# beast-dev/beast-mcmc

Hardware: NVIDIA H100
Metric: tree log-likelihood evals/sec (higher is better)
Workload: dtype f64

## Files before the change

beast-mcmc_b200/csrc/api.cu:

```cuda
#include "../../include/libhmsbeagle_b200.h"
#include "engine.h"
#include "multi.h"

#include <algorithm>
#include <atomic>
#include <chrono>
#include <cmath>
#include <cstdio>
#include <cstdlib>
#include <cstring>
#include <string>
#include <unordered_map>

using namespace b200;

namespace {

std::mutex gMutex;
std::vector<Instance*> gInstances;

const long kSupportedFlags =
    BEAGLE_FLAG_PRECISION_DOUBLE | BEAGLE_FLAG_PRECISION_SINGLE | BEAGLE_FLAG_COMPUTATION_SYNCH | BEAGLE_FLAG_EIGEN_REAL |
    BEAGLE_FLAG_EIGEN_COMPLEX | BEAGLE_FLAG_SCALING_MANUAL | BEAGLE_FLAG_SCALING_DYNAMIC |
    BEAGLE_FLAG_SCALERS_RAW | BEAGLE_FLAG_SCALERS_LOG | BEAGLE_FLAG_VECTOR_NONE | BEAGLE_FLAG_THREADING_NONE |
    BEAGLE_FLAG_PROCESSOR_GPU | BEAGLE_FLAG_FRAMEWORK_CUDA | BEAGLE_FLAG_PARALLELOPS_GRID |
    BEAGLE_FLAG_PREORDER_TRANSPOSE_AUTO;

int envInt(const char* name, int dflt) {
    const char* v = getenv(name);
    return v ? atoi(v) : dflt;
}

int flushPending(Instance* in);

Instance* getInstance(int id) {
    std::lock_guard<std::mutex> lock(gMutex);
    if (id < 0 || id >= (int)gInstances.size()) return nullptr;
    return gInstances[id];
}

#define SH(id, expr)                                                                         \
    do {                                                                                     \
        Instance* p__ = getInstance(id);                                                     \
        if (p__ != nullptr && p__->shard != nullptr) {                                       \
            Sharded* sh = static_cast<Sharded*>(p__->shard);                                 \
            (void)sh;                                                                        \
            return (expr);                                                                   \
        }                                                                                    \
    } while (0)

#define GET_INSTANCE_LAZY(in, id)                                       \
    Instance* in = getInstance(id);                                     \
    if (in == nullptr) return BEAGLE_ERROR_UNINITIALIZED_INSTANCE;      \
    if (in->shard != nullptr) return BEAGLE_ERROR_NO_IMPLEMENTATION;    \
    if (cudaSetDevice(in->device) != cudaSuccess) return BEAGLE_ERROR_GENERAL;

#define GET_INSTANCE(in, id)                                            \
    GET_INSTANCE_LAZY(in, id)                                           \
    if (!in->pendingMats.empty() || !in->pendingOps.empty()) {          \
        const int flushRc__ = flushPending(in);                         \
        if (flushRc__ != BEAGLE_SUCCESS) return flushRc__;              \
    }

#define CUDA_OK(expr)                                                                        \
    do {                                                                                     \
        cudaError_t e__ = (expr);                                                            \
        if (e__ != cudaSuccess) {                                                            \
            if (getenv("B200_BEAGLE_DEBUG"))                                                 \
                fprintf(stderr, "[b200-beagle] %s failed: %s (%s:%d)\n", #expr,              \
                        cudaGetErrorString(e__), __FILE__, __LINE__);                        \
            return e__ == cudaErrorMemoryAllocation ? BEAGLE_ERROR_OUT_OF_MEMORY             \
                                                    : BEAGLE_ERROR_GENERAL;                  \
        }                                                                                    \
    } while (0)

struct TimedScope {
    Instance* in;
    int cls;
    cudaEvent_t a = nullptr, b = nullptr;
    TimedScope(Instance* i, int c, int kernels = 1) : in(i), cls(c) {
        if (in->timing) {
            in->timedLaunches[cls] += kernels - 1;
            cudaEventCreate(&a);
            cudaEventCreate(&b);
            cudaEventRecord(a, in->stream);
        }
    }
    ~TimedScope() {
        if (in->timing) {
            cudaEventRecord(b, in->stream);
            in->timed[cls].push_back({a, b});
        }
    }
};

void* stage(Instance* in, const void* src, size_t bytes) {
    size_t need = (bytes + 255) & ~size_t(255);
    if (need > in->stageSize) return nullptr;
    if (in->stagePos + need > in->stageSize) {
        cudaStreamSynchronize(in->stream);
        in->stagePos = 0;
    }
    char* h = in->hStage + in->stagePos;
    char* d = in->dStage + in->stagePos;
    memcpy(h, src, bytes);
    if (cudaMemcpyAsync(d, h, bytes, cudaMemcpyHostToDevice, in->stream) != cudaSuccess) return nullptr;
    in->stagePos += need;
    return d;
}

int uploadSmall(Instance* in, void* dDst, const void* src, size_t bytes) {
    size_t need = (bytes + 255) & ~size_t(255);
    if (need > in->stageSize) return BEAGLE_ERROR_OUT_OF_RANGE;
    if (in->stagePos + need > in->stageSize) {
        cudaStreamSynchronize(in->stream);
        in->stagePos = 0;
    }
    char* h = in->hStage + in->stagePos;
    memcpy(h, src, bytes);
    in->stagePos += need;
    CUDA_OK(cudaMemcpyAsync(dDst, h, bytes, cudaMemcpyHostToDevice, in->stream));
    return BEAGLE_SUCCESS;
}

char* ensurePartials(Instance* in, int idx) {
    if (in->partials[idx] == nullptr) {
        if (in->nextSlot >= in->nSlots) return nullptr;
        in->slotOf[idx] = in->nextSlot++;
        in->partials[idx] = in->partialsBase + (size_t)in->slotOf[idx] * in->partialsElems * in->elemBytes();
    }
    return in->partials[idx];
}

bool validRange(int idx, int n) { return idx >= 0 && idx < n; }

void destroyInstance(Instance* in) {
    if (in->shard != nullptr) { shardedDestroy(in); delete in; return; }
    cudaSetDevice(in->device);
    exchangeRelease(in);
    if (in->stream) cudaStreamSynchronize(in->stream);
    cudaFree(in->partialsBase); cudaFree(in->states8Base); cudaFree(in->states32Base);
    for (CachedPlan& cp : in->planCache) { cp.dropGraph(); cudaFree(cp.dBlock); }
    cudaFree(in->dEigen); cudaFree(in->dMat); cudaFree(in->dEvec); cudaFree(in->dIncSums); cudaFree(in->dIncCounter);
    cudaFree(in->dRecipe);
    if (in->hMapped) cudaFreeHost(in->hMapped); cudaFree(in->dRates); cudaFree(in->dWeights);
    cudaFree(in->dFreqs); cudaFree(in->dScale); cudaFree(in->dPatternWeights);
    cudaFree(in->dPatternPartitions); cudaFree(in->dSite); cudaFree(in->dBlockSums); cudaFree(in->dOut);
    cudaFree(in->dCounter); cudaFree(in->dStage); cudaFree(in->dScratch);
    if (in->hStage) cudaFreeHost(in->hStage);
    if (in->hOut) cudaFreeHost(in->hOut);
    for (int c = 0; c < T_CLASSES; ++c)
        for (auto& ev : in->timed[c]) { cudaEventDestroy(ev.first); cudaEventDestroy(ev.second); }
    if (in->stream) cudaStreamDestroy(in->stream);
    delete in;
}

std::vector<BeagleResource> gResources;
std::vector<int> gShardDevices;
int gShardResource = -1;
std::vector<std::string> gResourceStrings;
BeagleResourceList gResourceList = {nullptr, 0};
std::once_flag gResourceOnce;

void buildResources() {
    int n = 0;
    if (cudaGetDeviceCount(&n) != cudaSuccess) { cudaGetLastError(); n = 0; }
    gResourceStrings.reserve(2 * (n + 1));
    gResourceStrings.push_back("CPU (host)");
    gResourceStrings.push_back("no host implementation in this library | use a GPU resource (1..N)");
    for (int d = 0; d < n; ++d) {
        cudaDeviceProp prop;
        if (cudaGetDeviceProperties(&prop, d) != cudaSuccess) { cudaGetLastError(); continue; }
        char buf[512];
        snprintf(buf, sizeof buf, "%s", prop.name);
        gResourceStrings.push_back(buf);
        snprintf(buf, sizeof buf, "Global memory (MB): %zu | SMs: %d | compute capability: %d.%d | "
                 "native walk kernels (sm_90a), fp64 arithmetic, fp64 or fp32 (4-state) partials",
                 (size_t)(prop.totalGlobalMem >> 20), prop.multiProcessorCount, prop.major, prop.minor);
        gResourceStrings.push_back(buf);
    }
    gShardDevices.clear();
    if (const char* env = getenv("B200_SHARD_DEVICES")) {
        for (const char* q = env; *q;) {
            char* end = nullptr;
            const long d = strtol(q, &end, 10);
            if (end == q) break;
            if (d >= 0 && d < n) gShardDevices.push_back((int)d);
            q = (*end == ',') ? end + 1 : end;
        }
    } else {
        for (int d = 0; d < n; ++d) gShardDevices.push_back(d);
    }
    if (gShardDevices.size() > (size_t)kMaxGroup) gShardDevices.resize(kMaxGroup);
    if (!gShardDevices.empty()) {
        char buf[512];
        snprintf(buf, sizeof buf, "GPU x %zu (pattern-sharded)", gShardDevices.size());
        gResourceStrings.push_back(buf);
        snprintf(buf, sizeof buf, "one instance over %zu GPUs | contiguous pattern blocks (Patterns.java:142-169 rule) | "
                 "per-shard sums added over NVLink inside the root kernel", gShardDevices.size());
        gResourceStrings.push_back(buf);
        gShardResource = (int)(gResourceStrings.size() / 2) - 1;
    }
    size_t count = gResourceStrings.size() / 2;
// ... 966 lines not shown
    in->planCache.reserve(16);
    in->thinR1 = envInt("B200_THIN_R1", 1);
    in->stackTail = envInt("B200_STACK_TAIL", 0);
    in->phaseT = envInt("B200_PHASE_T", 0);
    in->phaseTmin = std::max(1, envInt("B200_PHASE_TMIN", 4));
    in->phaseSmall = envInt("B200_PHASE_SMALL", 24);
    in->phaseOversub = std::max(0, envInt("B200_PHASE_OVERSUB", 0));
    in->walkMinBlocks = envInt("B200_WALK_MINB", 4);
    in->walkMinBlocksSet = getenv("B200_WALK_MINB") != nullptr;
    in->tensorR = envInt("B200_TENSOR_R", 2) >= 4 ? 4 : 2;
    in->genericMma = envInt("B200_GENERIC_MMA", 1);
    in->mmaWarps = envInt("B200_MMA_WARPS", 4) == 8 ? 8 : 4;
    cudaDeviceProp prop;
    bool ok = cudaGetDeviceProperties(&prop, in->device) == cudaSuccess;
    if (ok) { in->smCount = prop.multiProcessorCount; in->maxSmemOptin = prop.sharedMemPerBlockOptin; }
    in->walkR = envInt("B200_WALK_R", 4);
    if (in->walkR != 1 && in->walkR != 2 && in->walkR != 4 && in->walkR != 8) in->walkR = 4;
    if (getenv("B200_WALK_R") == nullptr && in->matCP > 0) {
        const int G = 32 / in->matCP;
        while (in->walkR > 1 && (in->Ppad + G * in->walkR - 1) / (G * in->walkR) < in->smCount) in->walkR >>= 1;
    }
    in->stackDepthMax = std::min(64, std::max(0, envInt("B200_STACK_DEPTH", 12)));
    if (single) { in->walkVariant = 0; in->stackTail = 0; }

    ok = ok && cudaStreamCreateWithFlags(&in->stream, cudaStreamNonBlocking) == cudaSuccess;
    const size_t eigenStride = 2 * (size_t)in->S * in->S + 2 * in->S;
    const size_t matElems = (size_t)in->nMatrices * in->matStride;
    const int rootBlocks = (in->Ppad + 255) / 256;
    in->stageSize = size_t(8) << 20;
    auto alloc = [&](auto** p, size_t elems) {
        if (!ok) return;
        using T = std::remove_pointer_t<std::remove_pointer_t<decltype(p)>>;
        size_t bytes = std::max<size_t>(elems, 1) * sizeof(T);
        ok = cudaMalloc(reinterpret_cast<void**>(p), bytes) == cudaSuccess &&
             cudaMemsetAsync(*p, 0, bytes, in->stream) == cudaSuccess;
    };
    alloc(&in->dEigen, std::max(1, in->nEigen) * eigenStride);
    alloc(&in->dMat, matElems);
    if (in->matCP > 0) alloc(&in->dEvec, (size_t)in->nMatrices * in->matCP * 4);
    if (in->matCP > 0 && in->matCP <= 8 && in->virtualCherries) {
        alloc(&in->dRecipe, (size_t)in->nBuffers * 32 * in->matCP);
        in->cherryTip1.assign(in->nBuffers, -1);
        in->cherryTip2.assign(in->nBuffers, -1);
        in->cherryStored.assign(in->nBuffers, 0);
    }
    if (in->matCP > 0 && in->matCP <= 8) {
        alloc(&in->dIncSums, (size_t)in->Ppad / 4 + 8);
        alloc(&in->dIncCounter, 4);
        in->fuseSmall = envInt("B200_FUSE", 1);
        if (ok && in->fuseSmall) {
            if (cudaHostAlloc(reinterpret_cast<void**>(&in->hMapped), 64, cudaHostAllocMapped) == cudaSuccess &&
                cudaHostGetDevicePointer(reinterpret_cast<void**>(&in->dMapped), in->hMapped, 0) == cudaSuccess) {
                memset(in->hMapped, 0, 64);
            } else {
                cudaGetLastError();
                if (in->hMapped) cudaFreeHost(in->hMapped);
                in->hMapped = nullptr;
            }
        }
    }
    alloc(&in->dRates, (size_t)in->nSets * in->C);
    alloc(&in->dWeights, (size_t)in->nSets * in->C);
    alloc(&in->dFreqs, (size_t)in->nSets * in->Sp);
    alloc(&in->dScale, (size_t)in->nScale * in->Ppad);
    alloc(&in->dPatternWeights, in->Ppad);
    alloc(&in->dPatternPartitions, in->Ppad);
    alloc(&in->dSite, in->Ppad);
    alloc(&in->dBlockSums, rootBlocks);
    alloc(&in->dOut, 1024);
    alloc(&in->dCounter, 4);
    alloc(&in->dStage, in->stageSize);
    alloc(&in->states8Base, (size_t)std::max(1, in->tipCount) * in->Ppad);
    alloc(&in->states32Base, (size_t)std::max(1, in->tipCount) * in->Ppad);
    if (ok) {
        int want[2] = {in->nPartials, std::max(1, in->nPartials - std::min(in->nCompact, in->tipCount))};
        for (int attempt = 0; attempt < 2 && in->partialsBase == nullptr; ++attempt) {
            size_t bytes = (size_t)want[attempt] * in->partialsElems * in->elemBytes();
            if (cudaMalloc(reinterpret_cast<void**>(&in->partialsBase), bytes) == cudaSuccess) in->nSlots = want[attempt];
            else { cudaGetLastError(); in->partialsBase = nullptr; }
        }
        if (in->partialsBase == nullptr) { destroyInstance(in); return BEAGLE_ERROR_OUT_OF_MEMORY; }
    }
    ok = ok && cudaMallocHost(reinterpret_cast<void**>(&in->hStage), in->stageSize) == cudaSuccess;
    ok = ok && cudaMallocHost(reinterpret_cast<void**>(&in->hOut), 1024 * sizeof(double)) == cudaSuccess;
    if (ok) {
        in->hRates.assign((size_t)in->nSets * in->C, 1.0);
        in->hWeights.assign((size_t)in->nSets * in->C, 0.0);
        in->hFreqs.assign((size_t)in->nSets * 4, 0.0);
        std::vector<double> ones((size_t)std::max(in->nSets * in->C, in->Ppad), 1.0);
        ok = cudaMemcpyAsync(in->dRates, ones.data(), sizeof(double) * in->nSets * in->C, cudaMemcpyHostToDevice,
                             in->stream) == cudaSuccess;
        std::vector<double> w(in->Ppad, 0.0);
        std::fill(w.begin(), w.begin() + in->P, 1.0);
        ok = ok && cudaMemcpyAsync(in->dPatternWeights, w.data(), sizeof(double) * in->Ppad, cudaMemcpyHostToDevice,
                                   in->stream) == cudaSuccess;
        ok = ok && cudaStreamSynchronize(in->stream) == cudaSuccess;
    }
    if (!ok) {
        cudaError_t e = cudaGetLastError();
        destroyInstance(in);
        return e == cudaErrorMemoryAllocation ? BEAGLE_ERROR_OUT_OF_MEMORY : BEAGLE_ERROR_GENERAL;
    }
    in->partitionCount = 1;
    in->partBegin.assign(1, 0);
    in->partEnd.assign(1, in->P);
    {
        std::lock_guard<std::mutex> lock(gMutex);
        int id = -1;
        for (size_t k = 0; k < gInstances.size(); ++k) if (gInstances[k] == nullptr) { id = (int)k; break; }
        if (id < 0) { gInstances.push_back(nullptr); id = (int)gInstances.size() - 1; }
        gInstances[id] = in;
        in->id = id;
    }
    if (returnInfo != nullptr) {
        returnInfo->resourceNumber = resource;
        returnInfo->resourceName = rl->list[resource].name;
        returnInfo->implName = single ? gImplNameSingle : gImplName;
        returnInfo->implDescription = gImplDesc;
        returnInfo->flags = in->flags;
    }
    return in->id;
}

int beagleFinalizeInstance(int instance) {
    Instance* in = nullptr;
    {
        std::lock_guard<std::mutex> lock(gMutex);
        if (instance < 0 || instance >= (int)gInstances.size() || gInstances[instance] == nullptr)
            return BEAGLE_ERROR_UNINITIALIZED_INSTANCE;
        in = gInstances[instance];
        gInstances[instance] = nullptr;
    }
    destroyInstance(in);
    return BEAGLE_SUCCESS;
}

int beagleFinalize(void) {
    std::vector<Instance*> all;
    {
        std::lock_guard<std::mutex> lock(gMutex);
        all.swap(gInstances);
    }
    for (Instance* in : all) if (in) destroyInstance(in);
    return BEAGLE_SUCCESS;
}

int beagleSetCPUThreadCount(int instance, int) {
    SH(instance, BEAGLE_SUCCESS);
    GET_INSTANCE(in, instance);
    (void)in;
    return BEAGLE_SUCCESS;
}

int beagleSetTipStates(int instance, int tipIndex, const int* inStates) {
    SH(instance, shSetTipStates(sh, tipIndex, inStates));
    GET_INSTANCE(in, instance);
    if (!validRange(tipIndex, in->nBuffers) || inStates == nullptr) return BEAGLE_ERROR_OUT_OF_RANGE;
    std::vector<int> s32(in->Ppad, in->S);
    std::vector<uint8_t> s8(in->Ppad, (uint8_t)in->S);
    for (int p = 0; p < in->P; ++p) {
        int s = inStates[p];
        if (s < 0 || s >= in->S) s = in->S;
        s32[p] = s;
        s8[p] = (uint8_t)s;
    }
    if (tipIndex >= in->tipCount) return BEAGLE_ERROR_OUT_OF_RANGE;
// ... 141 lines not shown
    GET_INSTANCE(in, instance);
    if (!validRange(stateFrequenciesIndex, in->nSets)) return BEAGLE_ERROR_OUT_OF_RANGE;
    std::vector<double> f(in->Sp, 0.0);
    memcpy(f.data(), inStateFrequencies, sizeof(double) * in->S);
    if (in->hFreqs.size() == (size_t)in->nSets * 4 && in->S <= 4)
        for (int i = 0; i < 4; ++i) in->hFreqs[(size_t)stateFrequenciesIndex * 4 + i] = i < in->S ? inStateFrequencies[i] : 0.0;
    return uploadSmall(in, in->dFreqs + (size_t)stateFrequenciesIndex * in->Sp, f.data(), sizeof(double) * in->Sp);
}

int beagleSetCategoryWeights(int instance, int categoryWeightsIndex, const double* inCategoryWeights) {
    SH(instance, shBroadcast(sh, [&](int c) { return beagleSetCategoryWeights(c, categoryWeightsIndex, inCategoryWeights); }));
    GET_INSTANCE(in, instance);
    if (!validRange(categoryWeightsIndex, in->nSets)) return BEAGLE_ERROR_OUT_OF_RANGE;
    std::copy(inCategoryWeights, inCategoryWeights + in->C, in->hWeights.begin() + (size_t)categoryWeightsIndex * in->C);
    return uploadSmall(in, in->dWeights + (size_t)categoryWeightsIndex * in->C, inCategoryWeights, sizeof(double) * in->C);
}

int beagleSetCategoryRatesWithIndex(int instance, int categoryRatesIndex, const double* inCategoryRates) {
    SH(instance, shBroadcast(sh, [&](int c) { return beagleSetCategoryRatesWithIndex(c, categoryRatesIndex, inCategoryRates); }));
    GET_INSTANCE(in, instance);
    if (!validRange(categoryRatesIndex, in->nSets)) return BEAGLE_ERROR_OUT_OF_RANGE;
    std::copy(inCategoryRates, inCategoryRates + in->C, in->hRates.begin() + (size_t)categoryRatesIndex * in->C);
    return uploadSmall(in, in->dRates + (size_t)categoryRatesIndex * in->C, inCategoryRates, sizeof(double) * in->C);
}

int beagleSetCategoryRates(int instance, const double* inCategoryRates) {
    return beagleSetCategoryRatesWithIndex(instance, 0, inCategoryRates);
}

int beagleSetPatternWeights(int instance, const double* inPatternWeights) {
    SH(instance, shSetPatternWeights(sh, inPatternWeights));
    GET_INSTANCE(in, instance);
    std::vector<double> w(in->Ppad, 0.0);
    memcpy(w.data(), inPatternWeights, sizeof(double) * in->P);
    CUDA_OK(cudaMemcpyAsync(in->dPatternWeights, w.data(), sizeof(double) * in->Ppad, cudaMemcpyHostToDevice, in->stream));
    CUDA_OK(cudaStreamSynchronize(in->stream));
    return BEAGLE_SUCCESS;
}

int beagleSetPatternPartitions(int instance, int partitionCount, const int* inPatternPartitions) {
    SH(instance, BEAGLE_ERROR_NO_IMPLEMENTATION);
    GET_INSTANCE(in, instance);
    if (partitionCount < 1 || partitionCount > 1000) return BEAGLE_ERROR_OUT_OF_RANGE;
    std::vector<int> begin(partitionCount, 0), end(partitionCount, 0);
    int prev = -1;
    for (int p = 0; p < in->P; ++p) {
        int k = inPatternPartitions[p];
        if (k < 0 || k >= partitionCount) return BEAGLE_ERROR_OUT_OF_RANGE;
        if (k < prev) return BEAGLE_ERROR_NO_IMPLEMENTATION;
        if (k != prev) { for (int q = prev + 1; q <= k; ++q) begin[q] = end[q] = p; prev = k; }
        end[k] = p + 1;
    }
    for (int q = prev + 1; q < partitionCount; ++q) begin[q] = end[q] = in->P;
    in->bufferEpoch++;
    in->partitionCount = partitionCount;
    in->partBegin = begin;
    in->partEnd = end;
    in->hostPartitions.assign(inPatternPartitions, inPatternPartitions + in->P);
    return BEAGLE_SUCCESS;
}

static int updateMatricesImpl(Instance* in, const int* eigenIndices, int eigenIndexScalar, const int* rateSets,
                              const int* probabilityIndices, const double* edgeLengths, int count) {
    if (count <= 0) return BEAGLE_SUCCESS;
    std::vector<double> block((size_t)count + (3 * (size_t)count + 1) / 2);
    int* pack = reinterpret_cast<int*>(block.data() + count);
    for (int k = 0; k < count; ++k) {
        int e = eigenIndices ? eigenIndices[k] : eigenIndexScalar;
        int r = rateSets ? rateSets[k] : 0;
        if (!validRange(probabilityIndices[k], in->nMatrices) || !validRange(e, in->nEigen) ||
            !validRange(r, in->nSets))
            return BEAGLE_ERROR_OUT_OF_RANGE;
        pack[k] = probabilityIndices[k];
        pack[count + k] = e;
        pack[2 * (size_t)count + k] = r;
    }
    if (in->matCP > 0)
        for (int k = 0; k < count; ++k) {
            const int e = eigenIndices ? eigenIndices[k] : eigenIndexScalar;
            in->matEigen[probabilityIndices[k]] = e;
            in->matEigenGen[probabilityIndices[k]] = in->eigenGen[e];
        }
    memcpy(block.data(), edgeLengths, sizeof(double) * count);
    double* dLen = static_cast<double*>(stage(in, block.data(), sizeof(double) * block.size()));
    if (dLen == nullptr) return BEAGLE_ERROR_OUT_OF_MEMORY;
    int* dIdx = reinterpret_cast<int*>(dLen + count);
    TimedScope ts(in, T_MATRICES);
    CUDA_OK(launchTransitionMatrices(in, dIdx, dIdx + count, dIdx + 2 * (size_t)count, dLen, count));
    return BEAGLE_SUCCESS;
}

}
namespace {
int flushPendingImpl(Instance* in) {
    int rc = BEAGLE_SUCCESS;
    if (!in->pendingMats.empty()) {
        const int n = (int)in->pendingMats.size();
        std::vector<int> eig(n), rate(n), prob(n);
        std::vector<double> len(n);
        for (int k = 0; k < n; ++k) {
            eig[k] = in->pendingMats[k].eigen; rate[k] = in->pendingMats[k].rateSet;
            prob[k] = in->pendingMats[k].prob; len[k] = in->pendingMats[k].len;
        }
        in->pendingMats.clear();
        rc = updateMatricesImpl(in, eig.data(), 0, rate.data(), prob.data(), len.data(), n);
    }
    if (!in->pendingOps.empty()) {
        std::vector<HostOp> hops;
        hops.swap(in->pendingOps);
        const int rc2 = planAndLaunch(in, hops, false);
        if (rc == BEAGLE_SUCCESS) rc = rc2;
    }
    return rc;
}

bool fusionPossible(const Instance* in) {
    return in->fuseSmall && in->matCP > 0 && in->matCP <= 8 && !in->timing && !in->exchangeOn && in->walkVariant == 0 &&
           in->eigenWalk && in->hMapped != nullptr;
}

int launchFused(Instance* in, int E, int wIdx, int fIdx, int cum, double* outSum) {
    IncArgs A;
    memset(&A, 0, sizeof A);
    A.partials = in->partialsBase; A.stride = in->partialsElems; A.states = in->states8Base; A.mats = in->dMat;
    A.evecs = in->dEvec; A.scale = in->dScale; A.matStride = in->matStride;
    A.S = in->S; A.C = in->C; A.Ppad = in->Ppad; A.P = in->P; A.logScalers = in->logScalers ? 1 : 0;
    const double* h = in->hEigen.data() + (size_t)E * 36;
    for (int q = 0; q < 16; ++q) { A.V[q] = h[q]; A.Vi[q] = h[16 + q]; }
    for (int q = 0; q < 4; ++q) A.eval[q] = h[32 + q];
    A.nMats = (int)in->pendingMats.size();
    std::unordered_map<int, int> pendingOf;
    for (int q = 0; q < A.nMats; ++q) {
        A.mat[q] = IncMat{in->pendingMats[q].prob, in->pendingMats[q].rateSet, in->pendingMats[q].len};
        for (int c = 0; c < 8; ++c) A.rate[q][c] = c < in->C ? in->hRates[(size_t)in->pendingMats[q].rateSet * in->C + c] : 0.0;
        pendingOf[in->pendingMats[q].prob] = q;
    }
    A.nOps = (int)in->pendingOps.size();
    {
        std::vector<int> outside;
        for (int k = 0; k < A.nOps; ++k)
            for (int c : {in->pendingOps[k].c1, in->pendingOps[k].c2}) {
                bool written = false;
                for (int w = 0; w < k; ++w) written = written || in->pendingOps[w].dest == c;
                if (!written) outside.push_back(c);
            }
        CUDA_OK(storeCherries(in, outside.data(), (int)outside.size()));
    }
    int prevDest = -1;
    for (int k = 0; k < A.nOps; ++k) {
        const HostOp& o = in->pendingOps[k];
        IncOp& d = A.op[k];
        const bool t1 = in->states32[o.c1] != nullptr, t2 = in->states32[o.c2] != nullptr;
        int c1 = o.c1, c2 = o.c2, m1 = o.m1, m2 = o.m2;
        d.flags = 0;
        if (k > 0 && !t1 && c1 == prevDest) d.flags = 1;
        else if (k > 0 && !t2 && c2 == prevDest) { std::swap(c1, c2); std::swap(m1, m2); d.flags = 1; }
        const bool s1 = in->states32[c1] != nullptr, s2 = in->states32[c2] != nullptr;
        d.dest = in->slotOf[o.dest];
        d.c1 = s1 ? -(c1 + 1) : in->slotOf[c1];
        d.c2 = s2 ? -(c2 + 1) : in->slotOf[c2];
        auto mat = [&](int m) { auto it = pendingOf.find(m); return it == pendingOf.end() ? m : -(it->second + 1); };
        d.m1 = mat(m1); d.m2 = mat(m2);
        d.sw = o.sw; d.sr = o.sw >= 0 ? -1 : o.sr;
        prevDest = o.dest;
    }
    for (int c = 0; c < 8; ++c) A.weights[c] = c < in->C ? in->hWeights[(size_t)wIdx * in->C + c] : 0.0;
    for (int i = 0; i < 4; ++i) A.freqs[i] = in->hFreqs[(size_t)fIdx * 4 + i];
    A.cum = cum == BEAGLE_OP_NONE ? nullptr : in->dScale + (size_t)cum * in->Ppad;
    A.patternWeights = in->dPatternWeights; A.site = in->dSite; A.blockSums = in->dIncSums; A.counter = in->dIncCounter;
// ... 988 lines not shown
```

beast-mcmc_b200/csrc/engine.h:

```cpp
#pragma once
#include <cuda_runtime.h>
#include <cstdint>
#include <mutex>
#include <vector>

namespace b200 {

struct alignas(16) DevOp {
    double* dest;
    const double* c1;
    const double* c2;
    const void* s1;
    const void* s2;
    const double* m1;
    const double* m2;
    double* scaleWrite;
    const double* scaleRead;
    double* cumScale;
    int pBegin, pEnd;
    int srcSlot1, srcSlot2;
    int dstSlot;
    int pad_;
};

// ... 57 lines not shown
    double* site; double* blockSums; unsigned int* counter; double* out;
    volatile double* hostOut; volatile unsigned long long* hostFlag; unsigned long long seq;
    IncMat mat[kIncMaxMats];
    IncOp op[kIncMaxOps];
};

constexpr int kMaxGroup = 16;
struct ExchangeSlot { double value; unsigned long long seq; };
struct Exchange {
    int rank = 0, size = 1;
    unsigned long long seq = 0;
    long long timeoutCycles = 0;
    ExchangeSlot* peers[kMaxGroup] = {};
};

constexpr int kStackSlots = 3;

struct Instance {
    int id = -1, device = 0, resource = 0;
    int tipCount = 0, nPartials = 0, nCompact = 0, S = 0, P = 0, nEigen = 0, nMatrices = 0, C = 0, nScale = 0;
    int Sp = 0, Ppad = 0, nBuffers = 0, nSets = 1;
    long flags = 0;
    bool logScalers = false, complexEigen = false;
    cudaStream_t stream = nullptr;
    int smCount = 132;
    size_t maxSmemOptin = 0;

    bool single = false;
    size_t partialsElems = 0;
    size_t elemBytes() const { return single ? sizeof(float) : sizeof(double); }
    char* partialsBase = nullptr;
    int nSlots = 0, nextSlot = 0;
    std::vector<int> slotOf;
    std::vector<char*> partials;
    uint8_t* states8Base = nullptr;
    int* states32Base = nullptr;
    std::vector<uint8_t*> states8;
    std::vector<int*> states32;
    int matCP = 0;
    size_t matStride = 0;

    double* dEigen = nullptr;
    double* dMat = nullptr;
    double* dEvec = nullptr;
    std::vector<int> matEigen;
    std::vector<unsigned> matEigenGen, eigenGen;
    std::vector<char> eigenReal;
    std::vector<char> eigenKind;
    std::vector<double> hEigen;
    int eigenWalk = 1;
    int tipMode = 2;
    int thinTipMode = 3;
    int virtualCherries = 1;
    std::vector<int> cherryTip1, cherryTip2;
    std::vector<char> cherryStored;
    double* dRecipe = nullptr;
    double* dRates = nullptr;
    std::vector<double> hRates, hWeights, hFreqs;
    double* dWeights = nullptr;
    double* dFreqs = nullptr;
    double* dScale = nullptr;
    std::vector<char> scaleIsLog;
    double* dPatternWeights = nullptr;
    int* dPatternPartitions = nullptr;
    double* dSite = nullptr;
    double* dBlockSums = nullptr;
    double* dOut = nullptr;
    unsigned int* dCounter = nullptr;
    int lookaheadPre = 1;
    int prePhases = 1;
    int useGraphs = 1;
    int lookahead = 1;
    int forward = 1;
    int stackSlots = kStackSlots;
    bool debugLog = false;
    double* dScratch = nullptr;
    size_t scratchDoubles = 0;
    int partitionCount = 1;
    std::vector<int> partBegin, partEnd;
    std::vector<int> hostPartitions;

    char* hStage = nullptr;
    char* dStage = nullptr;
    size_t stageSize = 0, stagePos = 0;
    double* hOut = nullptr;

    int fuseSmall = 1;
    struct PendingMat { int prob, eigen, rateSet; double len; };
    std::vector<PendingMat> pendingMats;
    std::vector<HostOp> pendingOps;
    int pendingCum = -1;
    double* hMapped = nullptr;
    double* dMapped = nullptr;
    double* dIncSums = nullptr;
    unsigned int* dIncCounter = nullptr;
    unsigned long long incSeq = 0;
    long fusedLaunches = 0;

    void* shard = nullptr;
    Exchange exchange;
    ExchangeSlot* dSlots = nullptr;
    std::vector<void*> ipcOpened;
    bool exchangeOn = false;

    bool timing = false;
    std::vector<std::pair<cudaEvent_t, cudaEvent_t>> timed[T_CLASSES];
    double timedMs[T_CLASSES] = {0, 0, 0};
    long timedLaunches[T_CLASSES] = {0, 0, 0};

    size_t walkSmemConfigured = 0, genericSmemConfigured = 0, mmaSmemConfigured[8] = {0, 0, 0, 0, 0, 0, 0, 0};
    int walkBlock = 128;
    int walkVariant = 0;
    std::vector<CachedPlan> planCache;
    int planCacheSize = 4;
    long planClock = 0;
    unsigned long bufferEpoch = 0;
    int reorder = 1;
    int thinR1 = 1;
    int stackTail = 0;
    int stackDepthMax = 12;
    int walkMinBlocks = 4;
    bool walkMinBlocksSet = false;
    int mmaWarps = 4;
    int tensorR = 2;
    int genericMma = 1;
    int walkR = 4;
    int phaseTmin = 4, phaseOversub = 0, phaseSmall = 24;
    int phaseT = 0;
};

struct Sharded;
Instance* instanceById(int id);
void exchangeRelease(Instance* in);
int shardedCreate(Instance* parent, int g, const int* devices, int tipCount, int partialsBufferCount, int compactBufferCount,
                  int stateCount, int patternCount, int eigenBufferCount, int matrixBufferCount, int categoryCount,
                  int scaleBufferCount, long preferenceFlags, long requirementFlags, void* details );
void shardedDestroy(Instance* parent);

cudaError_t launchTransitionMatrices(Instance* in, const int* dProbIdx, const int* dEigenIdx,
                                     const int* dRateSet, const double* dLengths, int count);
cudaError_t launchWalk4(Instance* in, const Op4* dOps, const int4* dSubs, int nSubs, int stackDepth, int maxWindow, bool preOrder);
cudaError_t updateWalk4EGraph(cudaGraphExec_t exec, const std::vector<cudaGraphNode_t>& kernelNodes, const double* eigen);
cudaError_t launchWalk4E(Instance* in, const Op4* dOps, const int4* dSubs, int nSubs, int maxWindow, bool aligned,
                         const double* eigen, const int4* dVirtTips, int stackSlots);
bool walk4pServes(const Instance* in, int nSubs, int maxWindow);
bool walkStackBuilt(const Instance* in);
cudaError_t launchCherrySnapshot(Instance* in, const int4* dItems, int count);
cudaError_t launchCherryStore(Instance* in, const int4* dItems, int count);
cudaError_t launchWalkGeneric(Instance* in, const DevOp* dOps, const int4* dSubs, int nSubs, int maxWindow, bool preOrder);
size_t edgeDerivativeWorkspace(const Instance* in, int count);
cudaError_t launchEdgeDerivatives(Instance* in, const EdgeRefT<void>* dEdges, int count, const double* weights, double* outPerPattern,
                                  double* outSum, double* outSumSq, double* partial);
int compressSitePatterns(int device, int taxa, int sites, const int* hStates, int* hPatternOfSite, int* hPatterns,
                         double* hWeights, int* hPatternCount);
int crossProductBlocks(const Instance* in, int count);
cudaError_t launchCrossProducts(Instance* in, const EdgeRefT<void>* dEdges, int count, const double* rates,
                                const double* weights, double* scratch);
cudaError_t launchRoot(Instance* in, const void* root, const double* weights, const double* freqs,
                       const double* cumScale, int pBegin, int pEnd, double* dOutSlot, const Exchange* exchange = nullptr);
cudaError_t launchIncremental(Instance* in, const IncArgs& args);
cudaError_t launchCombineMatrices(Instance* in, const int* dFirst, const int* dSecond, const int* dResult, int count, bool multiply);
cudaError_t launchExchangeSum(Instance* in, const double* dVals, int n, double* dOutJoint, const Exchange* exchange);
cudaError_t launchScaleAccumulate(Instance* in, const int* dIdx, int count, double* cum, double sign,
                                  int pBegin, int pEnd);
cudaError_t launchRescalePartialsForGet(Instance* in, double* tmp, const double* cum);

// ... 45 lines not shown
```

beast-mcmc_b200/csrc/kernels.cu:

```cuda
#include "engine.h"
#include "walk4.cuh"

#include <algorithm>
#include <cfloat>

namespace b200 {

__device__ __forceinline__ void dmma884acc(double& d0, double& d1, double a, double b) {
    asm("mma.sync.aligned.m8n8k4.row.col.f64.f64.f64.f64 {%0,%1}, {%2}, {%3}, {%0,%1};"
        : "+d"(d0), "+d"(d1) : "d"(a), "d"(b));
}

__global__ void k_transition(const double* __restrict__ eigenBase, size_t eigenStride, int S, int Sp, int C,
                             int complexForm, const double* __restrict__ ratesBase,
                             const int* __restrict__ probIdx, const int* __restrict__ eigenIdx,
                             const int* __restrict__ rateSet, const double* __restrict__ lengths,
                             double* __restrict__ matBase, size_t matStride, int matCP, double* __restrict__ evecBase) {
    extern __shared__ double sm[];
    double* ec = sm;
    double* ss = sm + S;
    int* pt = reinterpret_cast<int*>(sm + 2 * S);
    const int b = blockIdx.x, c = blockIdx.y;
    const double* E = eigenBase + (size_t)eigenIdx[b] * eigenStride;
    const double* evec = E;
    const double* ievc = E + (size_t)S * S;
    const double* eval = E + 2 * (size_t)S * S;
    const double d = lengths[b] * ratesBase[(size_t)rateSet[b] * C + c];
    for (int k = threadIdx.x; k < S; k += blockDim.x) {
        double im = complexForm ? eval[S + k] : 0.0;
        if (im == 0.0) {
            ec[k] = exp(d * eval[k]); ss[k] = 0.0; pt[k] = k;
        } else {
            int run = 0;
            for (int q = k - 1; q >= 0 && eval[S + q] != 0.0; --q) ++run;
            const bool first = (run % 2 == 0);
            int k0 = first ? k : k - 1;
            double bb = eval[S + k0];
            double expat = exp(d * eval[k0]);
            ec[k] = expat * cos(d * bb);
            ss[k] = (first ? 1.0 : -1.0) * expat * sin(d * bb);
            pt[k] = first ? k + 1 : k - 1;
        }
    }
    __syncthreads();
    if (evecBase != nullptr && threadIdx.x < 4)
        evecBase[((size_t)probIdx[b] * matCP + c) * 4 + threadIdx.x] = threadIdx.x < S ? ec[threadIdx.x] : 0.0;
    double* out = matBase + (size_t)probIdx[b] * matStride + (matCP ? (size_t)c * 4 : (size_t)c * Sp * Sp);
    const int rowStride = matCP ? matCP * 4 : Sp;
    for (int idx = threadIdx.x; idx < Sp * Sp; idx += blockDim.x) {
        int j = idx / Sp, i = idx % Sp;
        double acc = 0.0;
        if (i < S && j < S) {
            for (int k = 0; k < S; ++k) {
                double iexp = ec[k] * ievc[(size_t)k * S + j] + ss[k] * ievc[(size_t)pt[k] * S + j];
                acc += evec[(size_t)i * S + k] * iexp;
            }
            acc = fabs(acc);
        }
        out[(size_t)j * rowStride + i] = acc;
        if (!matCP) {
            const size_t ld = (size_t)Sp + 4;
            double* padded = matBase + (size_t)probIdx[b] * matStride + (size_t)C * Sp * Sp;
            padded[((size_t)c * Sp + i) * ld + j] = acc;
            padded[(size_t)C * Sp * ld + ((size_t)c * Sp + j) * ld + i] = acc;
        } else {
            double* mm = matBase + (size_t)probIdx[b] * matStride + 16 * matCP;
            mm[(size_t)c * 32 + i * 4 + j] = acc;
            mm[(size_t)c * 32 + 16 + i * 4 + j] = 0.0;
            double* mt = mm + (size_t)C * 32;
            mt[(size_t)c * 20 + j * 4 + i] = (j < S) ? acc : ((j == S && i < S) ? 1.0 : 0.0);
            if (j == 0) mt[(size_t)c * 20 + 16 + i] = (S == 4 && i < S) ? 1.0 : 0.0;
        }
    }
}

__device__ __forceinline__ size_t matEntry(int matCP, int Sp, int c, int i, int j) {
    return matCP ? ((size_t)j * matCP + c) * 4 + i : ((size_t)c * Sp + j) * Sp + i;
}
__global__ void __launch_bounds__(256)
k_combine_matrices(double* __restrict__ matBase, size_t matStride, int S, int Sp, int C, int matCP,
                   const int* __restrict__ first, const int* __restrict__ second, const int* __restrict__ result, int multiply) {
    const int q = blockIdx.x, c = blockIdx.y;
    const double* A = matBase + (size_t)first[q] * matStride;
    const double* B = matBase + (size_t)second[q] * matStride;
    double* R = matBase + (size_t)result[q] * matStride;
    for (int idx = threadIdx.x; idx < Sp * Sp; idx += blockDim.x) {
        const int i = idx / Sp, j = idx % Sp;
        double v = 0.0;
        if (i < S && j < S) {
            if (multiply) for (int k = 0; k < S; ++k) v += A[matEntry(matCP, Sp, c, i, k)] * B[matEntry(matCP, Sp, c, k, j)];
            else v = A[matEntry(matCP, Sp, c, i, j)] + B[matEntry(matCP, Sp, c, i, j)];
        }
        R[matEntry(matCP, Sp, c, i, j)] = v;
        if (!matCP) {
            const size_t ld = (size_t)Sp + 4;
            double* padded = R + (size_t)C * Sp * Sp;
            padded[((size_t)c * Sp + i) * ld + j] = v;
            padded[(size_t)C * Sp * ld + ((size_t)c * Sp + j) * ld + i] = v;
        } else {
            double* mm = R + 16 * matCP;
            mm[(size_t)c * 32 + i * 4 + j] = v;
            mm[(size_t)c * 32 + 16 + i * 4 + j] = 0.0;
            double* mt = mm + (size_t)C * 32;
            mt[(size_t)c * 20 + j * 4 + i] = (j < S) ? v : ((j == S && i < S) ? 1.0 : 0.0);
            if (j == 0) mt[(size_t)c * 20 + 16 + i] = (S == 4 && i < S) ? 1.0 : 0.0;
        }
    }
}

cudaError_t launchCombineMatrices(Instance* in, const int* dFirst, const int* dSecond, const int* dResult, int count, bool multiply) {
    if (count <= 0) return cudaSuccess;
    k_combine_matrices<<<dim3(count, in->C), 256, 0, in->stream>>>(in->dMat, in->matStride, in->S, in->Sp, in->C, in->matCP,
                                                                   dFirst, dSecond, dResult, multiply ? 1 : 0);
    return cudaGetLastError();
}

template <int NT>
__global__ void __launch_bounds__(128)
k_transition_mma(const double* __restrict__ eigenBase, size_t eigenStride, int S, int C,
                 const double* __restrict__ ratesBase, const int* __restrict__ probIdx,
                 const int* __restrict__ eigenIdx, const int* __restrict__ rateSet,
                 const double* __restrict__ lengths, double* __restrict__ matBase, size_t matStride) {
    constexpr int Sp = 8 * NT;
    constexpr int LD = Sp + 4;
    extern __shared__ double smt[];
    double* As = smt;
    double* Bt = smt + Sp * LD;
    double* ex = Bt + Sp * LD;
    const int b = blockIdx.x, c = blockIdx.y, tid = threadIdx.x;
    const double* E = eigenBase + (size_t)eigenIdx[b] * eigenStride;
    const double* evec = E;
    const double* ievc = E + (size_t)S * S;
    const double* eval = E + 2 * (size_t)S * S;
    const double d = lengths[b] * ratesBase[(size_t)rateSet[b] * C + c];
    for (int k = tid; k < Sp; k += 128) ex[k] = k < S ? exp(d * eval[k]) : 0.0;
    __syncthreads();
    for (int q = tid; q < Sp * Sp; q += 128) {
        const int r = q / Sp, col = q % Sp;
        As[r * LD + col] = (r < S && col < S) ? evec[(size_t)r * S + col] : 0.0;
        Bt[col * LD + r] = (r < S && col < S) ? ievc[(size_t)r * S + col] * ex[r] : 0.0;
    }
    __syncthreads();
    const int lane = tid & 31, w = tid >> 5, g = lane >> 2, t = lane & 3;
    double* outT = matBase + (size_t)probIdx[b] * matStride + (size_t)c * Sp * Sp;
    double* outR = matBase + (size_t)probIdx[b] * matStride + (size_t)C * Sp * Sp + (size_t)c * Sp * LD;
    double* outTp = outR + (size_t)C * Sp * LD;
    for (int mt = w; mt < NT; mt += 4) {
        double acc[NT][2];
#pragma unroll
        for (int n = 0; n < NT; ++n) { acc[n][0] = 0.0; acc[n][1] = 0.0; }
        const double* arow = As + (8 * mt + g) * LD + t;
        const double* brow = Bt + g * LD + t;
#pragma unroll 4
        for (int kc = 0; kc < Sp / 4; ++kc) {
            const double a = arow[4 * kc];
#pragma unroll
            for (int n = 0; n < NT; ++n) dmma884acc(acc[n][0], acc[n][1], a, brow[n * 8 * LD + 4 * kc]);
        }
        const int i = 8 * mt + g;
#pragma unroll
        for (int n = 0; n < NT; ++n) {
            const int j = 8 * n + 2 * t;
            const double v0 = fabs(acc[n][0]), v1 = fabs(acc[n][1]);
            *reinterpret_cast<double2*>(outR + (size_t)i * LD + j) = make_double2(v0, v1);
            outT[(size_t)j * Sp + i] = v0;
            outT[(size_t)(j + 1) * Sp + i] = v1;
            outTp[(size_t)j * LD + i] = v0;
            outTp[(size_t)(j + 1) * LD + i] = v1;
        }
    }
}

template <int NT>
static cudaError_t launchTransitionMmaT(Instance* in, const int* dProbIdx, const int* dEigenIdx, const int* dRateSet,
                                        const double* dLengths, int count) {
    constexpr int Sp = 8 * NT;
    const size_t smem = (2 * (size_t)Sp * (Sp + 4) + Sp) * sizeof(double);
    static_assert(Sp <= 64, "shared-memory budget");
    cudaError_t e = cudaFuncSetAttribute(k_transition_mma<NT>, cudaFuncAttributeMaxDynamicSharedMemorySize, (int)smem);
    if (e != cudaSuccess) return e;
    dim3 grid(count, in->C);
    k_transition_mma<NT><<<grid, 128, smem, in->stream>>>(in->dEigen, 2 * (size_t)in->S * in->S + 2 * in->S, in->S, in->C,
                                                          in->dRates, dProbIdx, dEigenIdx, dRateSet, dLengths, in->dMat,
                                                          in->matStride);
    return cudaGetLastError();
}

cudaError_t launchTransitionMatrices(Instance* in, const int* dProbIdx, const int* dEigenIdx,
                                     const int* dRateSet, const double* dLengths, int count) {
    if (count <= 0) return cudaSuccess;
    if (in->genericMma && in->matCP == 0 && !in->complexEigen) {
        switch (in->Sp / 8) {
            case 1: return launchTransitionMmaT<1>(in, dProbIdx, dEigenIdx, dRateSet, dLengths, count);
            case 2: return launchTransitionMmaT<2>(in, dProbIdx, dEigenIdx, dRateSet, dLengths, count);
            case 3: return launchTransitionMmaT<3>(in, dProbIdx, dEigenIdx, dRateSet, dLengths, count);
            case 4: return launchTransitionMmaT<4>(in, dProbIdx, dEigenIdx, dRateSet, dLengths, count);
            case 8: return launchTransitionMmaT<8>(in, dProbIdx, dEigenIdx, dRateSet, dLengths, count);
            default: break;
        }
    }
    size_t smem = (size_t)in->S * (2 * sizeof(double) + sizeof(int)) + 16;
    int threads = in->Sp * in->Sp >= 1024 ? 256 : (in->Sp * in->Sp >= 128 ? 128 : 32);
    dim3 grid(count, in->C);
    k_transition<<<grid, threads, smem, in->stream>>>(in->dEigen, 2 * (size_t)in->S * in->S + 2 * in->S, in->S,
                                                      in->Sp, in->C, in->complexEigen ? 1 : 0, in->dRates,
                                                      dProbIdx, dEigenIdx, dRateSet, dLengths, in->dMat,
                                                      in->matStride, in->matCP, in->matCP ? in->dEvec : nullptr);
    return cudaGetLastError();
}

struct Mat4 { double r[4][4]; };

template <int CP>
__device__ __forceinline__ void loadMat(const double* __restrict__ m, Mat4& M) {
    ldg256_ro(m, M.r[0]); ldg256_ro(m + 4 * CP, M.r[1]); ldg256_ro(m + 8 * CP, M.r[2]); ldg256_ro(m + 12 * CP, M.r[3]);
}

__device__ __forceinline__ void applyMat(const Mat4& M, const double (&x)[4], double (&y)[4]) {
#pragma unroll
    for (int i = 0; i < 4; ++i) y[i] = M.r[0][i] * x[0] + M.r[1][i] * x[1] + M.r[2][i] * x[2] + M.r[3][i] * x[3];
}

template <typename T, int CP, int R, bool STACK, bool FIRST>
__device__ __forceinline__ void childTerm(const WalkArgs& A, int child, int matIdx, int slot, int moff, size_t off0,
                                          int p0, bool catValid, int pBegin, int pEnd, const double2* stackMem,
                                          int nthreads, double (&y)[R][4]) {
    constexpr int G = 32 / CP;
    const int S = A.S;
    const double* m = A.mats + (size_t)matIdx * A.matStride + moff;
    if (child < 0) {
        const uint8_t* t = A.states + (size_t)(-child - 1) * A.Ppad;
#pragma unroll
        for (int r = 0; r < R; ++r) {
            const int p = p0 + r * G;
            const bool active = catValid && p >= pBegin && p < pEnd;
            const int s = active ? (int)__ldg(t + p) : S;
            double v[4];
            if (s < S) ldg256_ro(m + 4 * CP * s, v);
            else {
#pragma unroll
                for (int i = 0; i < 4; ++i) v[i] = (i < S) ? 1.0 : 0.0;
            }
#pragma unroll
            for (int i = 0; i < 4; ++i) y[r][i] = FIRST ? v[i] : y[r][i] * v[i];
        }
    } else {
        Mat4 M;
        loadMat<CP>(m, M);
        const T* xg = static_cast<const T*>(A.partials) + (size_t)child * A.stride + off0;
#pragma unroll
        for (int r = 0; r < R; ++r) {
            const int p = p0 + r * G;
            const bool active = catValid && p >= pBegin && p < pEnd;
            double x[4], v[4];
            if (STACK && slot != 0xFF) {
                double2 lo = stackMem[((slot * R + r) * 2 + 0) * nthreads + threadIdx.x];
                double2 hi = stackMem[((slot * R + r) * 2 + 1) * nthreads + threadIdx.x];
                x[0] = lo.x; x[1] = lo.y; x[2] = hi.x; x[3] = hi.y;
            } else if (active) {
                loadCell(xg + (size_t)r * G * 4, x);
            } else { x[0] = x[1] = x[2] = x[3] = 0.0; }
            applyMat(M, x, v);
#pragma unroll
            for (int i = 0; i < 4; ++i) y[r][i] = FIRST ? v[i] : y[r][i] * v[i];
        }
    }
}

template <typename T, int CP, int R, bool STACK, bool PRE>
__device__ __forceinline__ void walk4Body(const WalkArgs& A) {
    static_assert(sizeof(T) == 8 || !STACK, "the operand-stack variant is built for fp64 partials only");
    constexpr int G = 32 / CP;
    extern __shared__ double2 stackMem[];
    const int lane = threadIdx.x & 31;
    const int warp = (blockIdx.x * blockDim.x + threadIdx.x) >> 5;
    const int c = lane / G;
    const int4 range = __ldg(A.subs + blockIdx.y);
    const int p0 = range.z + warp * (G * R) + (lane % G);
    if (range.z + warp * (G * R) >= range.w) return;
    const bool catValid = c < A.C;
    const int cc = catValid ? c : 0;
    const size_t off0 = ((size_t)cc * A.Ppad + p0) * 4;
    const int moff = cc * 4;
    const int nthreads = blockDim.x;
    const int last = range.y - 1;

    Op4 cur = loadOp(A.ops + range.x);
    double d[R][4];
#pragma unroll
    for (int r = 0; r < R; ++r) d[r][0] = d[r][1] = d[r][2] = d[r][3] = 0.0;
// ... 1717 lines not shown
```

Before: 2578.

## Add quad-per-matrix transition kernel for 4-state compact layout and zero-copy index staging

Result: faster. 2666, median of 6 (+3.4%).

```diff
diff --git a/beast-mcmc_b200/csrc/api.cu b/beast-mcmc_b200/csrc/api.cu
--- a/beast-mcmc_b200/csrc/api.cu
+++ b/beast-mcmc_b200/csrc/api.cu
@@ -94,7 +94,7 @@
     }
 };
 
-void* stage(Instance* in, const void* src, size_t bytes) {
+static char* stageHost(Instance* in, const void* src, size_t bytes) {
     size_t need = (bytes + 255) & ~size_t(255);
     if (need > in->stageSize) return nullptr;
     if (in->stagePos + need > in->stageSize) {
@@ -102,23 +102,27 @@
         in->stagePos = 0;
     }
     char* h = in->hStage + in->stagePos;
-    char* d = in->dStage + in->stagePos;
-    memcpy(h, src, bytes);
-    if (cudaMemcpyAsync(d, h, bytes, cudaMemcpyHostToDevice, in->stream) != cudaSuccess) return nullptr;
-    in->stagePos += need;
-    return d;
-}
-
-int uploadSmall(Instance* in, void* dDst, const void* src, size_t bytes) {
-    size_t need = (bytes + 255) & ~size_t(255);
-    if (need > in->stageSize) return BEAGLE_ERROR_OUT_OF_RANGE;
-    if (in->stagePos + need > in->stageSize) {
-        cudaStreamSynchronize(in->stream);
-        in->stagePos = 0;
-    }
-    char* h = in->hStage + in->stagePos;
     memcpy(h, src, bytes);
     in->stagePos += need;
+    return h;
+}
+
+void* stage(Instance* in, const void* src, size_t bytes) {
+    char* h = stageHost(in, src, bytes);
+    if (h == nullptr) return nullptr;
+    char* d = in->dStage + (h - in->hStage);
+    if (cudaMemcpyAsync(d, h, bytes, cudaMemcpyHostToDevice, in->stream) != cudaSuccess) return nullptr;
+    return d;
+}
+
+static const void* stageMapped(Instance* in, const void* src, size_t bytes) {
+    char* h = stageHost(in, src, bytes);
+    return h == nullptr ? nullptr : in->hStageDev + (h - in->hStage);
+}
+
+int uploadSmall(Instance* in, void* dDst, const void* src, size_t bytes) {
+    char* h = stageHost(in, src, bytes);
+    if (h == nullptr) return BEAGLE_ERROR_OUT_OF_RANGE;
     CUDA_OK(cudaMemcpyAsync(dDst, h, bytes, cudaMemcpyHostToDevice, in->stream));
     return BEAGLE_SUCCESS;
 }
@@ -1251,6 +1255,7 @@
         if (in->partialsBase == nullptr) { destroyInstance(in); return BEAGLE_ERROR_OUT_OF_MEMORY; }
     }
     ok = ok && cudaMallocHost(reinterpret_cast<void**>(&in->hStage), in->stageSize) == cudaSuccess;
+    ok = ok && cudaHostGetDevicePointer(reinterpret_cast<void**>(&in->hStageDev), in->hStage, 0) == cudaSuccess;
     ok = ok && cudaMallocHost(reinterpret_cast<void**>(&in->hOut), 1024 * sizeof(double)) == cudaSuccess;
     if (ok) {
         in->hRates.assign((size_t)in->nSets * in->C, 1.0);
@@ -1558,9 +1563,11 @@
             in->matEigenGen[probabilityIndices[k]] = in->eigenGen[e];
         }
     memcpy(block.data(), edgeLengths, sizeof(double) * count);
-    double* dLen = static_cast<double*>(stage(in, block.data(), sizeof(double) * block.size()));
+    const size_t blockBytes = sizeof(double) * block.size();
+    const double* dLen = static_cast<const double*>(in->matCP > 0 ? stageMapped(in, block.data(), blockBytes)
+                                                                   : stage(in, block.data(), blockBytes));
     if (dLen == nullptr) return BEAGLE_ERROR_OUT_OF_MEMORY;
-    int* dIdx = reinterpret_cast<int*>(dLen + count);
+    const int* dIdx = reinterpret_cast<const int*>(dLen + count);
     TimedScope ts(in, T_MATRICES);
     CUDA_OK(launchTransitionMatrices(in, dIdx, dIdx + count, dIdx + 2 * (size_t)count, dLen, count));
     return BEAGLE_SUCCESS;
diff --git a/beast-mcmc_b200/csrc/engine.h b/beast-mcmc_b200/csrc/engine.h
--- a/beast-mcmc_b200/csrc/engine.h
+++ b/beast-mcmc_b200/csrc/engine.h
@@ -163,6 +163,7 @@
 
     char* hStage = nullptr;
     char* dStage = nullptr;
+    char* hStageDev = nullptr;
     size_t stageSize = 0, stagePos = 0;
     double* hOut = nullptr;
 
diff --git a/beast-mcmc_b200/csrc/kernels.cu b/beast-mcmc_b200/csrc/kernels.cu
--- a/beast-mcmc_b200/csrc/kernels.cu
+++ b/beast-mcmc_b200/csrc/kernels.cu
@@ -15,7 +15,7 @@
                              int complexForm, const double* __restrict__ ratesBase,
                              const int* __restrict__ probIdx, const int* __restrict__ eigenIdx,
                              const int* __restrict__ rateSet, const double* __restrict__ lengths,
-                             double* __restrict__ matBase, size_t matStride, int matCP, double* __restrict__ evecBase) {
+                             double* __restrict__ matBase, size_t matStride) {
     extern __shared__ double sm[];
     double* ec = sm;
     double* ss = sm + S;
@@ -43,10 +43,7 @@
         }
     }
     __syncthreads();
-    if (evecBase != nullptr && threadIdx.x < 4)
-        evecBase[((size_t)probIdx[b] * matCP + c) * 4 + threadIdx.x] = threadIdx.x < S ? ec[threadIdx.x] : 0.0;
-    double* out = matBase + (size_t)probIdx[b] * matStride + (matCP ? (size_t)c * 4 : (size_t)c * Sp * Sp);
-    const int rowStride = matCP ? matCP * 4 : Sp;
+    double* out = matBase + (size_t)probIdx[b] * matStride + (size_t)c * Sp * Sp;
     for (int idx = threadIdx.x; idx < Sp * Sp; idx += blockDim.x) {
         int j = idx / Sp, i = idx % Sp;
         double acc = 0.0;
@@ -57,21 +54,106 @@
             }
             acc = fabs(acc);
         }
-        out[(size_t)j * rowStride + i] = acc;
-        if (!matCP) {
-            const size_t ld = (size_t)Sp + 4;
-            double* padded = matBase + (size_t)probIdx[b] * matStride + (size_t)C * Sp * Sp;
-            padded[((size_t)c * Sp + i) * ld + j] = acc;
-            padded[(size_t)C * Sp * ld + ((size_t)c * Sp + j) * ld + i] = acc;
+        out[(size_t)j * Sp + i] = acc;
+        const size_t ld = (size_t)Sp + 4;
+        double* padded = matBase + (size_t)probIdx[b] * matStride + (size_t)C * Sp * Sp;
+        padded[((size_t)c * Sp + i) * ld + j] = acc;
+        padded[(size_t)C * Sp * ld + ((size_t)c * Sp + j) * ld + i] = acc;
+    }
+}
+
+constexpr int kTransition4Block = 256;
+__global__ void __launch_bounds__(kTransition4Block)
+k_transition4(const double* __restrict__ eigenBase, size_t eigenStride, int S, int C, int CP, int complexForm,
+              const double* __restrict__ ratesBase, const int* __restrict__ probIdx, const int* __restrict__ eigenIdx,
+              const int* __restrict__ rateSet, const double* __restrict__ lengths, int count,
+              double* __restrict__ matBase, size_t matStride, double* __restrict__ evecBase) {
+    constexpr int Q = kTransition4Block / 4;
+    __shared__ double sLen[Q];
+    __shared__ int sProb[Q], sEig[Q], sRate[Q];
+    const int lane = threadIdx.x & 31, k = lane & 3, i0 = 2 * (k & 1), j0 = 2 * (k >> 1);
+    const unsigned quad = 0xFu << (lane & ~3);
+    const int q = (int)(blockIdx.x * (unsigned)Q + (threadIdx.x >> 2));
+    const int bFirst = (int)(blockIdx.x * (unsigned)Q) / C;
+    const int nb = min(count, ((int)(blockIdx.x * (unsigned)Q) + Q - 1) / C + 1) - bFirst;
+    if ((int)threadIdx.x < nb) {
+        sLen[threadIdx.x] = lengths[bFirst + threadIdx.x];
+        sProb[threadIdx.x] = probIdx[bFirst + threadIdx.x];
+        sEig[threadIdx.x] = eigenIdx[bFirst + threadIdx.x];
+        sRate[threadIdx.x] = rateSet[bFirst + threadIdx.x];
+    }
+    __syncthreads();
+    if (q >= count * C) return;
+    const int b = q / C, c = q - b * C, r = b - bFirst;
+    const double* E = eigenBase + (size_t)sEig[r] * eigenStride;
+    const double* evec = E;
+    const double* ievc = E + (size_t)S * S;
+    const double* eval = E + 2 * (size_t)S * S;
+    const double d = __dmul_rn(sLen[r], ratesBase[(size_t)sRate[r] * C + c]);
+    double V[2][4], W[4][2];
+#pragma unroll
+    for (int m = 0; m < 4; ++m)
+#pragma unroll
+        for (int t = 0; t < 2; ++t) {
+            V[t][m] = (i0 + t < S && m < S) ? evec[(size_t)(i0 + t) * S + m] : 0.0;
+            W[m][t] = (m < S && j0 + t < S) ? ievc[(size_t)m * S + j0 + t] : 0.0;
+        }
+    double ec = 0.0, ss = 0.0;
+    int pt = k;
+    if (k < S) {
+        const double im = complexForm ? eval[S + k] : 0.0;
+        if (im == 0.0) {
+            ec = exp(__dmul_rn(d, eval[k]));
         } else {
-            double* mm = matBase + (size_t)probIdx[b] * matStride + 16 * matCP;
-            mm[(size_t)c * 32 + i * 4 + j] = acc;
-            mm[(size_t)c * 32 + 16 + i * 4 + j] = 0.0;
-            double* mt = mm + (size_t)C * 32;
-            mt[(size_t)c * 20 + j * 4 + i] = (j < S) ? acc : ((j == S && i < S) ? 1.0 : 0.0);
-            if (j == 0) mt[(size_t)c * 20 + 16 + i] = (S == 4 && i < S) ? 1.0 : 0.0;
-        }
-    }
+            int run = 0;
+            for (int m = k - 1; m >= 0 && eval[S + m] != 0.0; --m) ++run;
+            const bool first = (run % 2 == 0);
+            const int k0 = first ? k : k - 1;
+            const double bb = eval[S + k0];
+            const double expat = exp(__dmul_rn(d, eval[k0]));
+            ec = __dmul_rn(expat, cos(__dmul_rn(d, bb)));
+            ss = __dmul_rn(__dmul_rn(first ? 1.0 : -1.0, expat), sin(__dmul_rn(d, bb)));
+            pt = first ? k + 1 : k - 1;
+        }
+    }
+    double acc[2][2] = {{0.0, 0.0}, {0.0, 0.0}};
+#pragma unroll
+    for (int m = 0; m < 4; ++m) {
+        const double ecm = __shfl_sync(quad, ec, m, 4);
+        const double ssm = __shfl_sync(quad, ss, m, 4);
+        const int ptm = __shfl_sync(quad, pt, m, 4);
+        if (m < S) {
+#pragma unroll
+            for (int t = 0; t < 2; ++t) {
+                const double wp = (ptm == m || j0 + t >= S) ? W[m][t] : ievc[(size_t)ptm * S + j0 + t];
+                const double iexp = __fma_rn(ecm, W[m][t], __dmul_rn(ssm, wp));
+#pragma unroll
+                for (int a = 0; a < 2; ++a) acc[a][t] = __fma_rn(V[a][m], iexp, acc[a][t]);
+            }
+        }
+    }
+    double p[2][2], g[2][2];
+#pragma unroll
+    for (int a = 0; a < 2; ++a)
+#pragma unroll
+        for (int t = 0; t < 2; ++t) {
+            const int i = i0 + a, j = j0 + t;
+            p[a][t] = (i < S && j < S) ? fabs(acc[a][t]) : 0.0;
+            g[a][t] = (j < S) ? p[a][t] : ((j == S && i < S) ? 1.0 : 0.0);
+        }
+    const int mat = sProb[r];
+    double* base = matBase + (size_t)mat * matStride;
+    double* mm = base + 16 * (size_t)CP + (size_t)c * 32;
+    double* mt = base + 16 * (size_t)CP + (size_t)C * 32 + (size_t)c * 20;
+#pragma unroll
+    for (int t = 0; t < 2; ++t) {
+        *reinterpret_cast<double2*>(base + ((size_t)(j0 + t) * CP + c) * 4 + i0) = make_double2(p[0][t], p[1][t]);
+        *reinterpret_cast<double2*>(mt + (j0 + t) * 4 + i0) = make_double2(g[0][t], g[1][t]);
+        *reinterpret_cast<double2*>(mm + (i0 + t) * 4 + j0) = make_double2(p[t][0], p[t][1]);
+        *reinterpret_cast<double2*>(mm + 16 + 8 * t + 2 * k) = make_double2(0.0, 0.0);
+    }
+    mt[16 + k] = S == 4 ? 1.0 : 0.0;
+    evecBase[((size_t)mat * CP + c) * 4 + k] = k < S ? ec : 0.0;
 }
 
 __device__ __forceinline__ size_t matEntry(int matCP, int Sp, int c, int i, int j) {
@@ -189,7 +271,14 @@
 cudaError_t launchTransitionMatrices(Instance* in, const int* dProbIdx, const int* dEigenIdx,
                                      const int* dRateSet, const double* dLengths, int count) {
     if (count <= 0) return cudaSuccess;
-    if (in->genericMma && in->matCP == 0 && !in->complexEigen) {
+    if (in->matCP > 0) {
+        const unsigned blocks = (unsigned)(((size_t)count * in->C * 4 + kTransition4Block - 1) / kTransition4Block);
+        k_transition4<<<blocks, kTransition4Block, 0, in->stream>>>(in->dEigen, 2 * (size_t)in->S * in->S + 2 * in->S, in->S, in->C,
+                                                      in->matCP, in->complexEigen ? 1 : 0, in->dRates, dProbIdx, dEigenIdx,
+                                                      dRateSet, dLengths, count, in->dMat, in->matStride, in->dEvec);
+        return cudaGetLastError();
+    }
+    if (in->genericMma && !in->complexEigen) {
         switch (in->Sp / 8) {
             case 1: return launchTransitionMmaT<1>(in, dProbIdx, dEigenIdx, dRateSet, dLengths, count);
             case 2: return launchTransitionMmaT<2>(in, dProbIdx, dEigenIdx, dRateSet, dLengths, count);
@@ -205,7 +294,7 @@
     k_transition<<<grid, threads, smem, in->stream>>>(in->dEigen, 2 * (size_t)in->S * in->S + 2 * in->S, in->S,
                                                       in->Sp, in->C, in->complexEigen ? 1 : 0, in->dRates,
                                                       dProbIdx, dEigenIdx, dRateSet, dLengths, in->dMat,
-                                                      in->matStride, in->matCP, in->matCP ? in->dEvec : nullptr);
+                                                      in->matStride);
     return cudaGetLastError();
 }
 
```
